# lucidrains/audiolm-pytorch

Measured on NVIDIA H100. Metric: CoarseTransformer tokens/sec fwd+bwd seq2048, higher is better.
Workload: dtype bf16

## Files before the change

audiolm_pytorch_b200/_lib.py:

```python
from __future__ import annotations

import ctypes as C
import os
from pathlib import Path

import torch

_PKG = Path(__file__).resolve().parent
LIB_PATH = _PKG / "libalm_b200.so"

P = C.c_void_p
I = C.c_int
L = C.c_int64
F = C.c_float
U32 = C.c_uint32
U64 = C.c_uint64
DROP = [F, U64, U32]

SIGNATURES: dict[str, list] = {
    "alm_gemm_bf16": [P, I, L, L, P, I, L, L, P, I, L, L, I, I, I, I, F, P, I, I, P],
    "alm_mqa_attn_fwd": [P, L, P, L, L, P, L, L, P, P, L, P, L, P, L, L, I, I, I, I, I, F, *DROP, P],
    "alm_mqa_attn_bwd": [P, L, P, L, L, P, L, L, P, L, P, P, P, I, P, L, P, P, L, P, L, P, P, L, L, I, I, I, I, I, F, *DROP,
                         P],
    "alm_pack_key_mask": [P, P, I, I, P],
# ... 36 lines not shown
    "alm_rvq_pack_codebooks": [P, P, P, L, I, P],
    "alm_rvq_prepare": [P, L, P, P, L, P, I, I, P],
    "alm_rvq_select": [P, L, P, P, P, P, L, P, P, L, I, I, I, I, P],
    "alm_rvq_decode": [P, L, P, P, L, I, I, I, I, P],
}


class AlmError(RuntimeError):
    pass


_lib = None


def load() -> C.CDLL:
    global _lib
    if _lib is not None:
        return _lib
    if not LIB_PATH.exists():
        raise AlmError(
            f"{LIB_PATH} not found. Build it with `python -m audiolm_pytorch_b200.build` "
            "(there is no CPU / PyTorch fallback for the hot path)."
        )
    lib = C.CDLL(str(LIB_PATH), mode=os.RTLD_LOCAL | os.RTLD_NOW)
    lib.alm_version.restype = I
    lib.alm_status_string.restype = C.c_char_p
    lib.alm_status_string.argtypes = [I]
    lib.alm_launch_count.restype = C.c_ulonglong
    lib.alm_reset_launch_count.restype = None
    lib.alm_decode_stack_scratch_bytes.restype = L
    lib.alm_decode_stack_scratch_bytes.argtypes = [I, I, I, I]
    lib.alm_gemm_head_ce_tiles.restype = I
    lib.alm_gemm_head_ce_tiles.argtypes = [I]
    lib.alm_decode_stack_grid.restype = I
    lib.alm_decode_stack_grid.argtypes = []
    lib.alm_decode_stack_plan.restype = I
    lib.alm_decode_stack_plan.argtypes = [I, I, I, I, I, P]
    lib.alm_decode_stack_trace_offset.restype = L
    lib.alm_decode_stack_trace_offset.argtypes = [I, I, I, I]
    for name, argtypes in SIGNATURES.items():
        fn = getattr(lib, name)
        fn.argtypes = argtypes
        fn.restype = I
    _lib = lib
    return lib


def ptr(t) -> int | None:
    if t is None:
        return None
    return t.data_ptr()


def stream_handle() -> int:
    return torch.cuda.current_stream().cuda_stream


def call(name: str, *args) -> None:
    lib = load()
    conv = []
    for a in args:
        if isinstance(a, torch.Tensor):
            if not a.is_cuda:
                raise AlmError(f"{name}: got a {a.device} tensor; the hot path has no CPU implementation")
            conv.append(a.data_ptr())
        else:
# ... 13 lines not shown
```

audiolm_pytorch_b200/csrc/gemm_wgmma.cu:

```cuda
#include "alm_common.cuh"
#include "ptx_sm90.cuh"

namespace alm {

struct GemmParams {
  void* C;
  const float* bias;
  long long ldc, strideC;
  int M, N, K, batch;
  int m_blocks, n_blocks, k_blocks, split_k;
  int c_fp32, acc_mode;
  int tma_store;
  float alpha;
  int ce_mode;
  const long long* ce_labels;
  long long ce_ignore;
  float* ce_part;
  float* ce_lab;
  const float* ce_lse;
  const float* ce_num;
  const float* ce_den;
};

constexpr int GEMM_BLOCK_M = 128;
constexpr int GEMM_BLOCK_K = 64;
constexpr int GEMM_THREADS = 384;

template <int BLOCK_N>
struct GemmCfg {
  static constexpr int STAGES = BLOCK_N == 256 ? 4 : (BLOCK_N == 128 ? 6 : 8);
  static constexpr int A_BYTES = GEMM_BLOCK_M * GEMM_BLOCK_K * 2;
  static constexpr int B_BYTES = BLOCK_N * GEMM_BLOCK_K * 2;
  static constexpr int C_SUB_BYTES = 64 * 64 * 2;
  static constexpr int C_STAGE_BYTES = 4 * C_SUB_BYTES;
  static constexpr int SMEM_BYTES =
      STAGES * (A_BYTES + B_BYTES) + C_STAGE_BYTES + 1024  + 256 ;
  static_assert(SMEM_BYTES <= 227 * 1024, "exceeds the sm_90 dynamic shared memory limit");
};

template <int BLOCK_N, bool A_MN, bool B_MN, bool CE = false>
__global__ void __launch_bounds__(GEMM_THREADS, 1)
gemm_bf16_wgmma_kernel(const __grid_constant__ CUtensorMap tmA, const __grid_constant__ CUtensorMap tmB,
                       const __grid_constant__ CUtensorMap tmC, const GemmParams p) {
  using Cfg = GemmCfg<BLOCK_N>;
  constexpr int STAGES = Cfg::STAGES;
  extern __shared__ uint8_t smem_raw[];
  uint8_t* smem = reinterpret_cast<uint8_t*>((reinterpret_cast<uintptr_t>(smem_raw) + 1023) & ~uintptr_t(1023));
  uint8_t* smem_a = smem;
  uint8_t* smem_b = smem + STAGES * Cfg::A_BYTES;
  uint8_t* stage_c = smem + STAGES * (Cfg::A_BYTES + Cfg::B_BYTES);
  uint64_t* bars = reinterpret_cast<uint64_t*>(stage_c + Cfg::C_STAGE_BYTES);
  uint64_t* full_bar = bars;
  uint64_t* empty_bar = bars + STAGES;

  const int warp = threadIdx.x >> 5;
  const int lane = threadIdx.x & 31;
  const int wg = warp >> 2;

  if (threadIdx.x == 0) {
    tma_prefetch_desc(&tmA);
    tma_prefetch_desc(&tmB);
    if (p.tma_store) tma_prefetch_desc(&tmC);
    for (int i = 0; i < STAGES; ++i) {
      mbar_init(&full_bar[i], 1);
      mbar_init(&empty_bar[i], 8);
    }
    fence_mbar_init();
  }
  __syncthreads();

  const int tiles_per_batch = p.m_blocks * p.n_blocks * p.split_k;
  const int total_tiles = tiles_per_batch * p.batch;
  const int kb_per_split = (p.k_blocks + p.split_k - 1) / p.split_k;

  auto decode = [&](int t, int& b, int& s, int& mb, int& nb) {
    b = t / tiles_per_batch;
    int r = t - b * tiles_per_batch;
    s = r / (p.m_blocks * p.n_blocks);
    r -= s * (p.m_blocks * p.n_blocks);
    mb = r / p.n_blocks;
    nb = r - mb * p.n_blocks;
  };
  auto k_range = [&](int s, int& kb0, int& kb1) {
    kb0 = s * kb_per_split;
    kb1 = min(p.k_blocks, kb0 + kb_per_split);
  };

  if (wg == 0) {
    setmaxnreg_dec<40>();
    if (warp == 0) {
      int stage = 0;
      uint32_t phase = 0;
      for (int t = blockIdx.x; t < total_tiles; t += gridDim.x) {
        int b, s, mb, nb, kb0, kb1;
        decode(t, b, s, mb, nb);
        k_range(s, kb0, kb1);
        const int m0 = mb * GEMM_BLOCK_M, n0 = nb * BLOCK_N;
        for (int kb = kb0; kb < kb1; ++kb) {
          mbar_wait(&empty_bar[stage], phase ^ 1u);
          uint8_t* sa = smem_a + stage * Cfg::A_BYTES;
          uint8_t* sb = smem_b + stage * Cfg::B_BYTES;
          const int k0 = kb * GEMM_BLOCK_K;
          if (elect_one_sync()) {
            mbar_arrive_expect_tx(&full_bar[stage], Cfg::A_BYTES + Cfg::B_BYTES);
            if constexpr (!A_MN) {
              tma_load_3d(sa, &tmA, &full_bar[stage], k0, m0, b);
            } else {
#pragma unroll
              for (int i = 0; i < GEMM_BLOCK_M / 64; ++i)
                tma_load_3d(sa + i * (GEMM_BLOCK_K * 128), &tmA, &full_bar[stage], m0 + i * 64, k0, b);
            }
            if constexpr (!B_MN) {
              tma_load_3d(sb, &tmB, &full_bar[stage], k0, n0, b);
            } else {
#pragma unroll
              for (int i = 0; i < BLOCK_N / 64; ++i)
                tma_load_3d(sb + i * (GEMM_BLOCK_K * 128), &tmB, &full_bar[stage], n0 + i * 64, k0, b);
            }
          }
          __syncwarp();
          if (++stage == STAGES) { stage = 0; phase ^= 1u; }
        }
      }
    }
    return;
  }

  setmaxnreg_inc<232>();
  const int cw = wg - 1;
  const int wq = warp & 3;
  const int r_base = cw * 64 + wq * 16 + (lane >> 2);
  const int c_lane = 2 * (lane & 3);
  int stage = 0;
  uint32_t phase = 0;
  float acc[BLOCK_N / 2];
  for (int t = blockIdx.x; t < total_tiles; t += gridDim.x) {
    int b, s, mb, nb, kb0, kb1;
    decode(t, b, s, mb, nb);
    k_range(s, kb0, kb1);
    int prev_stage = -1;
    for (int kb = kb0; kb < kb1; ++kb) {
      mbar_wait(&full_bar[stage], phase);
      const uint32_t a_addr = smem_u32(smem_a + stage * Cfg::A_BYTES) + cw * 8192;
      const uint32_t b_addr = smem_u32(smem_b + stage * Cfg::B_BYTES);
      wgmma_fence_acc(acc);
      wgmma_fence();
#pragma unroll
      for (int k = 0; k < GEMM_BLOCK_K / 16; ++k) {
        const uint64_t da = A_MN ? wgmma_desc_sw128(a_addr + k * 2048, 1024, GEMM_BLOCK_K * 128)
                                 : wgmma_desc_sw128(a_addr + k * 32, 1024, 16);
        const uint64_t db = B_MN ? wgmma_desc_sw128(b_addr + k * 2048, 1024, GEMM_BLOCK_K * 128)
                                 : wgmma_desc_sw128(b_addr + k * 32, 1024, 16);
        wgmma_ss<BLOCK_N, A_MN ? 1 : 0, B_MN ? 1 : 0>(acc, da, db, (kb > kb0 || k > 0) ? 1u : 0u);
      }
      wgmma_commit();
      wgmma_wait<1>();
      wgmma_fence_acc(acc);
      if (prev_stage >= 0 && lane == 0) mbar_arrive(&empty_bar[prev_stage]);
      prev_stage = stage;
      if (++stage == STAGES) { stage = 0; phase ^= 1u; }
    }
    wgmma_wait<0>();
    wgmma_fence_acc(acc);
    if (prev_stage >= 0 && lane == 0) mbar_arrive(&empty_bar[prev_stage]);

    const int n0 = nb * BLOCK_N;
    if constexpr (!CE) {
      if (p.tma_store) {
        constexpr int SUBS = BLOCK_N / 64, NBUF = SUBS % 2 == 0 ? 2 : 1;
        const uint32_t st_base =
            smem_u32(stage_c) + cw * 2 * Cfg::C_SUB_BYTES + (wq * 16 + (lane >> 2)) * 128 + (lane & 3) * 4;
#pragma unroll
        for (int sub = 0; sub < SUBS; ++sub) {
          uint8_t* buf = stage_c + (cw * 2 + sub % NBUF) * Cfg::C_SUB_BYTES;
          if ((threadIdx.x & 127) == 0) bulk_wait_group_read<NBUF - 1>();
          named_bar_sync(1 + cw, 128);
#pragma unroll
          for (int h = 0; h < 2; ++h)
#pragma unroll
            for (int jj = 0; jj < 8; ++jj) {
              const int j = sub * 8 + jj;
              const int col = n0 + 8 * j + c_lane;
              float v0 = acc[4 * j + 2 * h] * p.alpha, v1 = acc[4 * j + 2 * h + 1] * p.alpha;
              if (p.bias != nullptr) {
                if (col < p.N) v0 += __ldg(p.bias + col);
                if (col + 1 < p.N) v1 += __ldg(p.bias + col + 1);
              }
              st_shared_u32(st_base + (sub % NBUF) * Cfg::C_SUB_BYTES + h * 1024 + ((jj ^ (lane >> 2)) << 4),
                            pack_bf16x2(v0, v1));
            }
          fence_proxy_async_smem();
          named_bar_sync(1 + cw, 128);
          if ((threadIdx.x & 127) == 0) {
            tma_store_3d(&tmC, buf, n0 + sub * 64, mb * GEMM_BLOCK_M + cw * 64, b);
            bulk_commit_group();
          }
        }
        continue;
      }
    }

#pragma unroll
    for (int h = 0; h < 2; ++h) {
      const int gm = mb * GEMM_BLOCK_M + r_base + 8 * h;
      const bool row_ok = gm < p.M;
      const long long row_off = (long long)b * p.strideC + (long long)gm * p.ldc;
      [[maybe_unused]] float ce_lse2 = 0.f, ce_scale = 0.f;
      [[maybe_unused]] long long ce_label = -1;
      if constexpr (CE) {
        if (row_ok) {
          ce_label = p.ce_labels[gm];
          if (p.ce_mode == 2) {
            ce_lse2 = p.ce_lse[gm] * 1.4426950408889634f;
            ce_scale = ce_label == p.ce_ignore ? 0.f : __ldg(p.ce_num) / __ldg(p.ce_den);
          }
        }
        if (p.ce_mode == 1) {
          float cm = -INFINITY;
#pragma unroll
          for (int j = 0; j < BLOCK_N / 8; ++j)
#pragma unroll
            for (int c = 0; c < 2; ++c) {
              const int col = n0 + 8 * j + c_lane + c;
              float v = acc[4 * j + 2 * h + c] * p.alpha;
              if (p.bias != nullptr && col < p.N) v += __ldg(p.bias + col);
              if (row_ok && col == ce_label) p.ce_lab[gm] = v;
              v = col < p.N ? v * 1.4426950408889634f : -INFINITY;
              acc[4 * j + 2 * h + c] = v;
              cm = fmaxf(cm, v);
            }
          cm = fmaxf(cm, __shfl_xor_sync(0xffffffffu, cm, 1));
          cm = fmaxf(cm, __shfl_xor_sync(0xffffffffu, cm, 2));
          float cs = 0.f;
#pragma unroll
          for (int j = 0; j < BLOCK_N / 8; ++j)
#pragma unroll
            for (int c = 0; c < 2; ++c) cs += exp2f(acc[4 * j + 2 * h + c] - cm);
          cs += __shfl_xor_sync(0xffffffffu, cs, 1);
          cs += __shfl_xor_sync(0xffffffffu, cs, 2);
          if (row_ok && (lane & 3) == 0) {
            float* pp = p.ce_part + ((size_t)gm * p.n_blocks + nb) * 2;
            pp[0] = cm;
            pp[1] = cs;
          }
          continue;
        }
      }
      if (!row_ok) continue;
#pragma unroll
      for (int j = 0; j < BLOCK_N / 8; ++j) {
        const int col = n0 + 8 * j + c_lane;
        if (col >= p.N) break;
        float v0 = acc[4 * j + 2 * h] * p.alpha, v1 = acc[4 * j + 2 * h + 1] * p.alpha;
        const bool pair = col + 1 < p.N;
        if (p.bias != nullptr) {
          v0 += __ldg(p.bias + col);
          if (pair) v1 += __ldg(p.bias + col + 1);
        }
        if constexpr (CE) {
          v0 = (exp2f(v0 * 1.4426950408889634f - ce_lse2) - (col == ce_label ? 1.f : 0.f)) * ce_scale;
          v1 = (exp2f(v1 * 1.4426950408889634f - ce_lse2) - (col + 1 == ce_label ? 1.f : 0.f)) * ce_scale;
        }
        if (p.c_fp32) {
          float* dst = reinterpret_cast<float*>(p.C) + row_off + col;
          const bool vec = pair && ((reinterpret_cast<uintptr_t>(dst) & 7u) == 0);
          if (p.acc_mode == 2) {
            if (vec) {
              asm volatile("red.global.add.v2.f32 [%0], {%1, %2};" ::"l"(dst), "f"(v0), "f"(v1) : "memory");
            } else {
              atomicAdd(dst, v0);
              if (pair) atomicAdd(dst + 1, v1);
            }
          } else if (vec) {
            float2 o = make_float2(v0, v1);
            if (p.acc_mode == 1) {
              const float2 old = *reinterpret_cast<float2*>(dst);
              o.x += old.x; o.y += old.y;
            }
            *reinterpret_cast<float2*>(dst) = o;
          } else {
            dst[0] = (p.acc_mode == 1 ? dst[0] : 0.f) + v0;
            if (pair) dst[1] = (p.acc_mode == 1 ? dst[1] : 0.f) + v1;
          }
        } else {
          __nv_bfloat16* dst = reinterpret_cast<__nv_bfloat16*>(p.C) + row_off + col;
          if (p.acc_mode != 0) {
            v0 += __bfloat162float(dst[0]);
            if (pair) v1 += __bfloat162float(dst[1]);
          }
          if (pair && ((reinterpret_cast<uintptr_t>(dst) & 3u) == 0)) {
            *reinterpret_cast<uint32_t*>(dst) = pack_bf16x2(v0, v1);
          } else {
            dst[0] = __float2bfloat16_rn(v0);
            if (pair) dst[1] = __float2bfloat16_rn(v1);
          }
        }
      }
    }
  }
  if ((threadIdx.x & 127) == 0) bulk_wait_group<0>();
}

template <int BLOCK_N, bool A_MN, bool B_MN, bool CE = false>
static int launch_gemm(const CUtensorMap& tmA, const CUtensorMap& tmB, const CUtensorMap& tmC, const GemmParams& p,
                       cudaStream_t stream) {
  using Cfg = GemmCfg<BLOCK_N>;
  auto kfn = gemm_bf16_wgmma_kernel<BLOCK_N, A_MN, B_MN, CE>;
  static bool attr_set = false;
  if (!attr_set) {
    ALM_CUDA_OK(cudaFuncSetAttribute(kfn, cudaFuncAttributeMaxDynamicSharedMemorySize, Cfg::SMEM_BYTES));
    attr_set = true;
  }
  const int total = p.m_blocks * p.n_blocks * p.split_k * p.batch;
  const int grid = total < num_sms() ? total : num_sms();
  kfn<<<grid, GEMM_THREADS, Cfg::SMEM_BYTES, stream>>>(tmA, tmB, tmC, p);
  ALM_CHECK_LAUNCH();
  ALM_LAUNCHED(1);
  return ALM_OK;
}

static int pick_block_n(int N) {
  if (N <= 64) return 64;
  if (N <= 128) return 128;
  const int pad256 = ceil_div(N, 256) * 256, pad128 = ceil_div(N, 128) * 128;
  return (pad128 * 10 < pad256 * 9) ? 128 : 256;
}

}

namespace alm {
struct CeEpilogue {
  int mode;
  const long long* labels;
  long long ignore;
  float* part;
  float* lab;
  const float* lse;
  const float* num;
  const float* den;
};
}

static int gemm_common(const void* A, int a_mn, int64_t lda, int64_t strideA, const void* B, int b_mn, int64_t ldb,
                       int64_t strideB, void* C, int c_fp32, int64_t ldc, int64_t strideC, int M, int N, int K, int batch,
                       float alpha, const float* bias, int acc_mode, int split_k, cudaStream_t stream,
                       const alm::CeEpilogue* ce) {
  using namespace alm;
  ALM_REQUIRE(A && B && (C || (ce && ce->mode == 1)), ALM_ERR_ARG);
  ALM_REQUIRE(M > 0 && N > 0 && K > 0 && batch > 0, ALM_ERR_ARG);
  ALM_REQUIRE(acc_mode >= 0 && acc_mode <= 2 && split_k >= 1, ALM_ERR_ARG);
  ALM_REQUIRE(split_k == 1 || (acc_mode == 2 && c_fp32), ALM_ERR_ARG);
  ALM_REQUIRE(!(a_mn && !b_mn), ALM_ERR_UNSUPPORTED);
  ALM_REQUIRE(lda % 8 == 0 && ldb % 8 == 0 && strideA % 8 == 0 && strideB % 8 == 0, ALM_ERR_ALIGN);

  const int BN = pick_block_n(N);
  GemmParams p;
  p.C = C;
  p.bias = bias;
  p.ldc = ldc;
  p.strideC = strideC;
  p.M = M; p.N = N; p.K = K; p.batch = batch;
  p.m_blocks = ceil_div(M, GEMM_BLOCK_M);
  p.n_blocks = ceil_div(N, BN);
  p.k_blocks = ceil_div(K, GEMM_BLOCK_K);
  if (split_k > p.k_blocks) split_k = p.k_blocks;
  while (split_k > 1 && (split_k - 1) * ceil_div(p.k_blocks, split_k) >= p.k_blocks) --split_k;
  p.split_k = split_k;
  p.c_fp32 = c_fp32;
  p.acc_mode = acc_mode;
  p.alpha = alpha;
  p.ce_mode = 0;
  if (ce != nullptr) {
    p.ce_mode = ce->mode;
    p.ce_labels = ce->labels;
    p.ce_ignore = ce->ignore;
    p.ce_part = ce->part;
    p.ce_lab = ce->lab;
    p.ce_lse = ce->lse;
    p.ce_num = ce->num;
    p.ce_den = ce->den;
  }

  CUtensorMap tmA, tmB;
  {
    uint64_t dims[3], strides[3];
    uint32_t box[3];
    if (!a_mn) {
      dims[0] = (uint64_t)K; dims[1] = (uint64_t)M;
      box[0] = GEMM_BLOCK_K; box[1] = GEMM_BLOCK_M;
    } else {
      dims[0] = (uint64_t)M; dims[1] = (uint64_t)K;
      box[0] = 64; box[1] = GEMM_BLOCK_K;
    }
    dims[2] = (uint64_t)batch; box[2] = 1;
    strides[0] = 2; strides[1] = (uint64_t)lda * 2;
    strides[2] = batch > 1 ? (uint64_t)strideA * 2 : dims[1] * strides[1];
    int rc = make_tensor_map(&tmA, A, 2, 3, dims, strides, box, true);
    if (rc != ALM_OK) return rc;
  }
  {
    uint64_t dims[3], strides[3];
    uint32_t box[3];
    if (!b_mn) {
      dims[0] = (uint64_t)K; dims[1] = (uint64_t)N;
      box[0] = GEMM_BLOCK_K; box[1] = (uint32_t)BN;
    } else {
      dims[0] = (uint64_t)N; dims[1] = (uint64_t)K;
      box[0] = 64; box[1] = GEMM_BLOCK_K;
    }
    dims[2] = (uint64_t)batch; box[2] = 1;
    strides[0] = 2; strides[1] = (uint64_t)ldb * 2;
    strides[2] = batch > 1 ? (uint64_t)strideB * 2 : dims[1] * strides[1];
    int rc = make_tensor_map(&tmB, B, 2, 3, dims, strides, box, true);
    if (rc != ALM_OK) return rc;
  }

  CUtensorMap tmC = {};
  p.tma_store = ce == nullptr && !c_fp32 && acc_mode == 0 && (reinterpret_cast<uintptr_t>(C) & 15u) == 0 &&
                (ldc * 2) % 16 == 0 && (batch == 1 || (strideC * 2) % 16 == 0);
  if (p.tma_store) {
    const uint64_t dims[3] = {(uint64_t)N, (uint64_t)M, (uint64_t)batch};
    const uint64_t strides[3] = {2, (uint64_t)ldc * 2, batch > 1 ? (uint64_t)strideC * 2 : (uint64_t)M * ldc * 2};
    const uint32_t box[3] = {64, 64, 1};
    int rc = make_tensor_map(&tmC, C, 2, 3, dims, strides, box, true);
    if (rc != ALM_OK) return rc;
  }

  if (ce != nullptr) {
    if (BN == 256) return launch_gemm<256, false, false, true>(tmA, tmB, tmC, p, stream);
    if (BN == 128) return launch_gemm<128, false, false, true>(tmA, tmB, tmC, p, stream);
    return launch_gemm<64, false, false, true>(tmA, tmB, tmC, p, stream);
  }
#define ALM_GEMM_DISPATCH(BN_)                                                             \
  if (!a_mn && !b_mn) return launch_gemm<BN_, false, false>(tmA, tmB, tmC, p, stream);     \
  if (!a_mn && b_mn) return launch_gemm<BN_, false, true>(tmA, tmB, tmC, p, stream);       \
  return launch_gemm<BN_, true, true>(tmA, tmB, tmC, p, stream);
  if (BN == 256) { ALM_GEMM_DISPATCH(256) }
  if (BN == 128) { ALM_GEMM_DISPATCH(128) }
  { ALM_GEMM_DISPATCH(64) }
#undef ALM_GEMM_DISPATCH
}

extern "C" int alm_gemm_bf16(const void* A, int a_mn, int64_t lda, int64_t strideA, const void* B, int b_mn,
                             int64_t ldb, int64_t strideB, void* C, int c_fp32, int64_t ldc, int64_t strideC, int M,
                             int N, int K, int batch, float alpha, const float* bias, int acc_mode, int split_k,
                             alm_stream_t stream_) {
  return gemm_common(A, a_mn, lda, strideA, B, b_mn, ldb, strideB, C, c_fp32, ldc, strideC, M, N, K, batch, alpha, bias,
                     acc_mode, split_k, reinterpret_cast<cudaStream_t>(stream_), nullptr);
}

extern "C" int alm_gemm_head_ce_tiles(int V) { return alm::ceil_div(V, alm::pick_block_n(V)); }

extern "C" int alm_gemm_head_ce(const void* X, int64_t ldx, const void* W, int64_t ldw, const float* bias,
                                const int64_t* labels, int64_t ignore_index, int mode, float* part, float* lab_logit,
                                const float* lse, const float* scale_num, const float* scale_den, void* dlogits,
                                int64_t ldd, int M, int V, int K, alm_stream_t stream_) {
  ALM_REQUIRE(mode == 1 || mode == 2, ALM_ERR_ARG);
  ALM_REQUIRE(labels != nullptr, ALM_ERR_ARG);
  if (mode == 1) ALM_REQUIRE(part && lab_logit, ALM_ERR_ARG);
  else ALM_REQUIRE(lse && scale_num && scale_den && dlogits && ldd >= V, ALM_ERR_ARG);
  alm::CeEpilogue ce{mode, reinterpret_cast<const long long*>(labels), (long long)ignore_index, part, lab_logit, lse,
                     scale_num, scale_den};
  return gemm_common(X, 0, ldx, 0, W, 0, ldw, 0, dlogits, 0, ldd, 0, M, V, K, 1, 1.f, bias, 0, 1,
                     reinterpret_cast<cudaStream_t>(stream_), &ce);
}
```

audiolm_pytorch_b200/csrc/ptx_sm90.cuh:

```cuda
#pragma once
#include <cuda.h>
#include <cuda_runtime.h>
#include <cuda_bf16.h>
#include <stdint.h>
#include <stdio.h>

namespace alm {

__device__ __forceinline__ uint32_t smem_u32(const void* p) {
  return static_cast<uint32_t>(__cvta_generic_to_shared(p));
}
__device__ __forceinline__ uint32_t lane_id() { return threadIdx.x & 31u; }

__device__ __forceinline__ uint64_t global_timer_ns() {
  uint64_t t;
  asm volatile("mov.u64 %0, %%globaltimer;" : "=l"(t));
  return t;
}

__device__ __forceinline__ void mbar_init(uint64_t* bar, uint32_t arrive_count) {
  asm volatile("mbarrier.init.shared::cta.b64 [%0], %1;" ::"r"(smem_u32(bar)), "r"(arrive_count) : "memory");
}
__device__ __forceinline__ void fence_mbar_init() {
  asm volatile("fence.mbarrier_init.release.cluster;" ::: "memory");
// ... 55 lines not shown
      ::"r"(smem_u32(smem_dst)), "l"(reinterpret_cast<uint64_t>(m)), "r"(smem_u32(bar)), "r"(c0), "r"(c1), "r"(c2)
      : "memory");
}
__device__ __forceinline__ void tma_store_3d(const CUtensorMap* m, const void* smem_src, int32_t c0, int32_t c1,
                                             int32_t c2) {
  asm volatile("cp.async.bulk.tensor.3d.global.shared::cta.bulk_group [%0, {%2, %3, %4}], [%1];"
               ::"l"(reinterpret_cast<uint64_t>(m)), "r"(smem_u32(smem_src)), "r"(c0), "r"(c1), "r"(c2)
               : "memory");
}
__device__ __forceinline__ void tma_reduce_add_3d(const CUtensorMap* m, uint32_t smem_src, int32_t c0, int32_t c1,
                                                  int32_t c2) {
  asm volatile("cp.reduce.async.bulk.tensor.3d.global.shared::cta.add.bulk_group [%0, {%2, %3, %4}], [%1];"
               ::"l"(reinterpret_cast<uint64_t>(m)), "r"(smem_src), "r"(c0), "r"(c1), "r"(c2)
               : "memory");
}
__device__ __forceinline__ void bulk_commit_group() { asm volatile("cp.async.bulk.commit_group;" ::: "memory"); }
template <int N>
__device__ __forceinline__ void bulk_wait_group_read() {
  asm volatile("cp.async.bulk.wait_group.read %0;" ::"n"(N) : "memory");
}
template <int N>
__device__ __forceinline__ void bulk_wait_group() {
  asm volatile("cp.async.bulk.wait_group %0;" ::"n"(N) : "memory");
}
__device__ __forceinline__ void st_shared_u32(uint32_t smem_addr, uint32_t v) {
  asm volatile("st.shared.u32 [%0], %1;" ::"r"(smem_addr), "r"(v) : "memory");
}
__device__ __forceinline__ void st_shared_f32x2(uint32_t smem_addr, float a, float b) {
  asm volatile("st.shared.v2.f32 [%0], {%1, %2};" ::"r"(smem_addr), "f"(a), "f"(b) : "memory");
}
__device__ __forceinline__ void named_bar_sync(uint32_t id, uint32_t nthreads) {
  asm volatile("bar.sync %0, %1;" ::"r"(id), "r"(nthreads) : "memory");
}
__device__ __forceinline__ uint64_t wgmma_desc_sw128(uint32_t smem_addr, uint32_t sbo_bytes, uint32_t lbo_bytes) {
  uint32_t lo = ((smem_addr >> 4) & 0x3FFFu) | (((lbo_bytes >> 4) & 0x3FFFu) << 16);
  uint32_t hi = ((sbo_bytes >> 4) & 0x3FFFu) | (1u << 30);
  return (static_cast<uint64_t>(hi) << 32) | lo;
}
__device__ __forceinline__ uint64_t wgmma_desc_nosw(uint32_t smem_addr, uint32_t sbo_bytes, uint32_t lbo_bytes) {
  uint32_t lo = ((smem_addr >> 4) & 0x3FFFu) | (((lbo_bytes >> 4) & 0x3FFFu) << 16);
  uint32_t hi = ((sbo_bytes >> 4) & 0x3FFFu);
  return (static_cast<uint64_t>(hi) << 32) | lo;
}
__device__ __forceinline__ void wgmma_fence() { asm volatile("wgmma.fence.sync.aligned;" ::: "memory"); }
__device__ __forceinline__ void wgmma_commit() { asm volatile("wgmma.commit_group.sync.aligned;" ::: "memory"); }
template <int N>
__device__ __forceinline__ void wgmma_wait() {
  asm volatile("wgmma.wait_group.sync.aligned %0;" ::"n"(N) : "memory");
}
template <int R>
__device__ __forceinline__ void wgmma_fence_acc(float (&d)[R]) {
#pragma unroll
  for (int i = 0; i < R; ++i) asm volatile("" : "+f"(d[i])::"memory");
}
template <int N>
__device__ __forceinline__ void setmaxnreg_inc() {
  asm volatile("setmaxnreg.inc.sync.aligned.u32 %0;" ::"n"(N));
}
template <int N>
__device__ __forceinline__ void setmaxnreg_dec() {
  asm volatile("setmaxnreg.dec.sync.aligned.u32 %0;" ::"n"(N));
}

template <int TA, int TB>
__device__ __forceinline__ void wgmma_ss_n32(float (&d)[16], uint64_t da, uint64_t db, uint32_t accumulate) {
  asm volatile(
// ... 103 lines not shown
```

audiolm_pytorch_b200/ops.py:

```python
from __future__ import annotations

import ctypes
import functools

import torch

from . import _lib

_SMS: dict[int, int] = {}


def num_sms(device=None) -> int:
    idx = None if device is None else torch.device(device).index
    if idx is None:
        idx = torch.cuda.current_device()
    if idx not in _SMS:
        _SMS[idx] = torch.cuda.get_device_properties(idx).multi_processor_count
    return _SMS[idx]


bf16 = torch.bfloat16
f32 = torch.float32


# ... 57 lines not shown
    assert a3.stride(-1) == 1 and b3.stride(-1) == 1
    nb = a3.shape[0]
    assert b3.shape[0] == nb
    if a_mn:
        K, M = a3.shape[1], a3.shape[2]
    else:
        M, K = a3.shape[1], a3.shape[2]
    if b_mn:
        Kb, N = b3.shape[1], b3.shape[2]
    else:
        N, Kb = b3.shape[1], b3.shape[2]
    assert K == Kb, f"K mismatch {K} vs {Kb}"
    if out is None:
        out = torch.empty((nb, M, N) if batched else (M, N), device=a.device, dtype=out_dtype)
        assert acc_mode == 0
    o3 = out.unsqueeze(0) if out.dim() == 2 else out
    assert o3.shape == (nb, M, N) and o3.stride(-1) == 1
    assert o3.dtype in (bf16, f32)
    if bias is not None:
        assert bias.dtype == f32 and bias.numel() == N and bias.is_contiguous()
    if _PROFILE is not None and PROFILE_SHAPES:
        cls += f" M{M} N{N} K{K} b{nb} {'mn' if a_mn else 'k'}{'mn' if b_mn else 'k'} s{split_k}"
    with _timed(cls, 2.0 * M * N * K * nb):
        _lib.call(
            "alm_gemm_bf16",
            a3, int(a_mn), a3.stride(1), a3.stride(0) if nb > 1 else 0,
            b3, int(b_mn), b3.stride(1), b3.stride(0) if nb > 1 else 0,
            o3, int(o3.dtype == f32), o3.stride(1), o3.stride(0) if nb > 1 else 0,
            M, N, K, nb, float(alpha), bias, int(acc_mode), int(split_k),
        )
    return out


def _check_bias(bias, heads, n_q, n_k):
    assert bias.dtype == f32 and bias.dim() == 3 and bias.shape[0] == heads and bias.shape[1] == n_q
    assert bias.shape[2] >= n_k and bias.stride(2) == 1 and bias.stride(1) % 4 == 0 and bias.stride(0) % 4 == 0
    return bias.stride(0), bias.stride(1)


def _ptr_array(tensors):
    import ctypes
    arr = (ctypes.c_void_p * len(tensors))(*[t.data_ptr() for t in tensors])
    return arr


def embed_gather(src, tables, d):
    _check_cuda(src, *tables)
    assert src.dtype == torch.int32 and src.is_contiguous() and src.shape[1] == 2
    assert all(t.dtype == f32 and t.is_contiguous() and t.shape[-1] == d for t in tables)
    M = src.shape[0]
    out = torch.empty(M, d, device=src.device, dtype=f32)
    import ctypes
    _lib.call("alm_embed_gather", ctypes.cast(_ptr_array(tables), ctypes.c_void_p), len(tables), src, out, M, d)
    return out


def embed_scatter(src, grad_tables, dout):
    _check_cuda(src, dout, *grad_tables)
    M, d = dout.shape
    assert dout.dtype == f32 and dout.is_contiguous()
    import ctypes
    _lib.call("alm_embed_scatter", ctypes.cast(_ptr_array(grad_tables), ctypes.c_void_p), len(grad_tables), src, dout,
              M, d)


class PackedKeyMask:
# ... 654 lines not shown
```

audiolm_pytorch_b200/transformer.py:

```python
from __future__ import annotations

import torch
from torch import nn

from . import ops

bf16 = torch.bfloat16
f32 = torch.float32


def exists(v):
    return v is not None


def default(v, d):
    return v if exists(v) else d


def _pad8(n: int) -> int:
    return (n + 7) // 8 * 8


def _check_dropout(p, name="dropout"):
    if not 0.0 <= float(p) < 1.0:
# ... 113 lines not shown
        self._cache = {}
        self.generation = 0

    def clear(self):
        self._cache.clear()
        self.generation += 1

    def get(self, key, params, build):
        ver = tuple((p.data_ptr(), p._version) for p in params)
        hit = self._cache.get(key)
        if hit is not None and hit[0] == ver:
            return hit[1]
        with torch.inference_mode(False), torch.no_grad():
            val = build()
        self._cache[key] = (ver, val)
        return val


def pack_plain(w):
    return ops.cast_pad(w.detach(), _pad8(w.shape[1]))


def pack_w1(w, inner):
    ip = _pad8(inner)
    out = torch.zeros(2 * ip, w.shape[1], device=w.device, dtype=bf16)
    ops.cast_pad(w.detach()[:inner], out=out[:inner])
    ops.cast_pad(w.detach()[inner:], out=out[ip:ip + inner])
    return out


def best_split_k(M, N, K, n_sm=None):
    if n_sm is None:
        n_sm = ops.num_sms() if torch.cuda.is_available() else 132
    bn = 64 if N <= 64 else (128 if N <= 128 or (-(-N // 128) * 128) * 10 < (-(-N // 256) * 256) * 9 else 256)
    tiles = -(-M // 128) * -(-N // bn)
    kb = -(-K // 64)
    best, best_t = 1, None
    for s in range(1, min(64, kb) + 1):
        t = -(-tiles * s // n_sm) * (-(-kb // s) + 6)
        if best_t is None or t < best_t:
            best, best_t = s, t
    return best


def wgrad(dy, x, out):
    Mtok = dy.shape[0]
    s = best_split_k(dy.shape[1], x.shape[1], Mtok)
    ops.gemm(dy, x, a_mn=True, b_mn=True, out=out, acc_mode=2 if s > 1 else 1, split_k=s)


class _StackFn(torch.autograd.Function):

    @staticmethod
    def forward(ctx, tr, x, mask, bias, drop, want_kv, *params):
        out, kv, saved = tr._walk_forward(x, mask, bias, drop, save=any(ctx.needs_input_grad), want_kv=want_kv)
        ctx.tr = tr
        ctx.saved = saved
        ctx.bias_grad = bias is not None and ctx.needs_input_grad[3]
        ctx.mark_non_differentiable(kv)
        return out, kv

    @staticmethod
    def backward(ctx, dout, _dkv):
        tr = ctx.tr
        S = ctx.saved
        S["dbias"] = torch.zeros_like(S["bias"]) if ctx.bias_grad else None
        dx, grads = tr._walk_backward(S, dout)
        dbias = S["dbias"]
        ctx.saved = None
        return (None, dx, None, dbias, None, None, *grads)


# ... 387 lines not shown
```

include/alm_b200.h:

```cpp
#ifndef ALM_B200_H_
#define ALM_B200_H_

#include <stddef.h>
#include <stdint.h>

#ifdef __cplusplus
extern "C" {
#endif

typedef struct CUstream_st* alm_stream_t;

typedef enum alm_status {
  ALM_OK = 0,
  ALM_ERR_ARG = -1,
  ALM_ERR_ALIGN = -2,
  ALM_ERR_CUDA = -3,
  ALM_ERR_UNSUPPORTED = -4
} alm_status;

int alm_version(void);
const char* alm_status_string(int code);
unsigned long long alm_launch_count(void);
void alm_reset_launch_count(void);

int alm_gemm_bf16(const void* A, int a_mn, int64_t lda, int64_t strideA, const void* B, int b_mn, int64_t ldb,
                  int64_t strideB, void* C, int c_fp32, int64_t ldc, int64_t strideC, int M, int N, int K, int batch,
                  float alpha, const float* bias, int acc_mode, int split_k, alm_stream_t stream);

int alm_embed_gather(const float* const* tables, int n_tables, const int32_t* src, float* out, int M, int d,
                     alm_stream_t stream);
int alm_embed_scatter(float* const* grad_tables, int n_tables, const int32_t* src, const float* dout, int M, int d,
                      alm_stream_t stream);
int alm_pack_key_mask(const void* key_mask, void* bits, int b, int n_k, alm_stream_t stream);
int alm_mqa_attn_fwd(const void* q, int64_t ldq, const void* k, int64_t ldk, int64_t k_bstride, const void* v,
                     int64_t ldv, int64_t v_bstride, const void* key_mask, void* o, int64_t ldo, float* lse,
                     int64_t lse_stride, const float* bias, int64_t bias_hstride, int64_t bias_rstride, int b, int h,
                     int n_q, int n_k, int causal, float scale, float dropout_p, uint64_t seed, uint32_t site,
                     alm_stream_t stream);

int alm_mqa_attn_bwd(const void* q, int64_t ldq, const void* k, int64_t ldk, int64_t k_bstride, const void* v,
                     int64_t ldv, int64_t v_bstride, const void* d_o, int64_t lddo, const void* key_mask,
                     const float* lse, const float* delta, int n_q_pad, void* dq, int64_t lddq, float* dq_acc,
                     void* dk, int64_t lddk, void* dv, int64_t lddv, const float* bias, float* dbias,
                     int64_t bias_hstride, int64_t bias_rstride, int b, int h, int n_q, int n_k, int causal,
                     float scale, float dropout_p, uint64_t seed, uint32_t site, alm_stream_t stream);
int alm_attn_delta(const void* o, int64_t ldo, const void* d_o, int64_t lddo, float* delta ,
                   int64_t delta_stride, float* dq_acc, int b, int h, int n, alm_stream_t stream);

int alm_bias_gather_fwd(const float* table, const int32_t* idx, const float* override_h, float* out, int heads,
                        int n_q, int n_k, int64_t ld, alm_stream_t stream);
int alm_bias_gather_bwd(const float* dbias, const int32_t* idx, float* dtable, float* doverride, int heads, int n_q,
                        int n_k, int64_t ld, alm_stream_t stream);

int alm_gemv_bf16(const void* x, int64_t ldx, const void* W, int64_t ldw, void* out, int c_fp32, int64_t ldo,
                  const float* bias, int rows, int N, int K, alm_stream_t stream);
int alm_kv_append(const void* kv_new, int64_t ld, void* k_cache, void* v_cache, int64_t cache_bstride,
                  const int32_t* len, int max_len, int b, alm_stream_t stream);
int alm_mqa_attn_decode(const void* q, int64_t ldq, const void* k_cache, const void* v_cache, int64_t cache_bstride,
                        const int32_t* len, int max_len, const void* key_mask, int64_t mask_bstride, const float* bias,
                        int64_t bias_ld, void* o, int64_t ldo,
// ... 105 lines not shown
```

Before: 752,800.

## Add ping-pong warpgroup GEMM variant for short-K bf16 TMA-store GEMMs

```diff
diff --git a/audiolm_pytorch_b200/_lib.py b/audiolm_pytorch_b200/_lib.py
--- a/audiolm_pytorch_b200/_lib.py
+++ b/audiolm_pytorch_b200/_lib.py
@@ -92,6 +92,10 @@
     lib.alm_decode_stack_scratch_bytes.argtypes = [I, I, I, I]
     lib.alm_gemm_head_ce_tiles.restype = I
     lib.alm_gemm_head_ce_tiles.argtypes = [I]
+    lib.alm_gemm_plan.restype = I
+    lib.alm_gemm_plan.argtypes = [I, I, I, I, I, P, P, P]
+    lib.alm_gemm_select_kernel.restype = I
+    lib.alm_gemm_select_kernel.argtypes = [I]
     lib.alm_decode_stack_grid.restype = I
     lib.alm_decode_stack_grid.argtypes = []
     lib.alm_decode_stack_plan.restype = I
diff --git a/audiolm_pytorch_b200/csrc/gemm_wgmma.cu b/audiolm_pytorch_b200/csrc/gemm_wgmma.cu
--- a/audiolm_pytorch_b200/csrc/gemm_wgmma.cu
+++ b/audiolm_pytorch_b200/csrc/gemm_wgmma.cu
@@ -38,10 +38,11 @@
   static_assert(SMEM_BYTES <= 227 * 1024, "exceeds the sm_90 dynamic shared memory limit");
 };
 
-template <int BLOCK_N, bool A_MN, bool B_MN, bool CE = false>
+template <int BLOCK_N, bool A_MN, bool B_MN, bool CE = false, bool PP = false>
 __global__ void __launch_bounds__(GEMM_THREADS, 1)
 gemm_bf16_wgmma_kernel(const __grid_constant__ CUtensorMap tmA, const __grid_constant__ CUtensorMap tmB,
                        const __grid_constant__ CUtensorMap tmC, const GemmParams p) {
+  static_assert(!PP || (BLOCK_N == 128 && !CE), "the ping-pong kernel has 128 x 128 tiles and no CE epilogue");
   using Cfg = GemmCfg<BLOCK_N>;
   constexpr int STAGES = Cfg::STAGES;
   extern __shared__ uint8_t smem_raw[];
@@ -63,7 +64,7 @@
     if (p.tma_store) tma_prefetch_desc(&tmC);
     for (int i = 0; i < STAGES; ++i) {
       mbar_init(&full_bar[i], 1);
-      mbar_init(&empty_bar[i], 8);
+      mbar_init(&empty_bar[i], PP ? 4 : 8);
     }
     fence_mbar_init();
   }
@@ -127,82 +128,110 @@
   }
 
   setmaxnreg_inc<232>();
+  constexpr int MH = PP ? 2 : 1;
   const int cw = wg - 1;
   const int wq = warp & 3;
-  const int r_base = cw * 64 + wq * 16 + (lane >> 2);
+  const int row0 = PP ? 0 : cw * 64;
+  const int r_base = row0 + wq * 16 + (lane >> 2);
   const int c_lane = 2 * (lane & 3);
   int stage = 0;
   uint32_t phase = 0;
-  float acc[BLOCK_N / 2];
-  for (int t = blockIdx.x; t < total_tiles; t += gridDim.x) {
+  float acc[MH][BLOCK_N / 2];
+  int i = 0;
+  for (int t = blockIdx.x; t < total_tiles; t += gridDim.x, ++i) {
     int b, s, mb, nb, kb0, kb1;
     decode(t, b, s, mb, nb);
     k_range(s, kb0, kb1);
+    if constexpr (PP) {
+      if ((i & 1) != cw) {
+        const int adv = stage + (kb1 - kb0);
+        phase ^= (uint32_t)(adv / STAGES) & 1u;
+        stage = adv % STAGES;
+        continue;
+      }
+      if (i > 0) named_bar_sync(3 + cw, 256);
+    }
     int prev_stage = -1;
     for (int kb = kb0; kb < kb1; ++kb) {
       mbar_wait(&full_bar[stage], phase);
-      const uint32_t a_addr = smem_u32(smem_a + stage * Cfg::A_BYTES) + cw * 8192;
+      const uint32_t a_addr = smem_u32(smem_a + stage * Cfg::A_BYTES) + row0 * 128;
       const uint32_t b_addr = smem_u32(smem_b + stage * Cfg::B_BYTES);
-      wgmma_fence_acc(acc);
+#pragma unroll
+      for (int mh = 0; mh < MH; ++mh) wgmma_fence_acc(acc[mh]);
       wgmma_fence();
 #pragma unroll
       for (int k = 0; k < GEMM_BLOCK_K / 16; ++k) {
-        const uint64_t da = A_MN ? wgmma_desc_sw128(a_addr + k * 2048, 1024, GEMM_BLOCK_K * 128)
-                                 : wgmma_desc_sw128(a_addr + k * 32, 1024, 16);
         const uint64_t db = B_MN ? wgmma_desc_sw128(b_addr + k * 2048, 1024, GEMM_BLOCK_K * 128)
                                  : wgmma_desc_sw128(b_addr + k * 32, 1024, 16);
-        wgmma_ss<BLOCK_N, A_MN ? 1 : 0, B_MN ? 1 : 0>(acc, da, db, (kb > kb0 || k > 0) ? 1u : 0u);
+#pragma unroll
+        for (int mh = 0; mh < MH; ++mh) {
+          const uint32_t am = a_addr + mh * 8192;
+          const uint64_t da = A_MN ? wgmma_desc_sw128(am + k * 2048, 1024, GEMM_BLOCK_K * 128)
+                                   : wgmma_desc_sw128(am + k * 32, 1024, 16);
+          wgmma_ss<BLOCK_N, A_MN ? 1 : 0, B_MN ? 1 : 0>(acc[mh], da, db, (kb > kb0 || k > 0) ? 1u : 0u);
+        }
       }
       wgmma_commit();
       wgmma_wait<1>();
-      wgmma_fence_acc(acc);
+#pragma unroll
+      for (int mh = 0; mh < MH; ++mh) wgmma_fence_acc(acc[mh]);
       if (prev_stage >= 0 && lane == 0) mbar_arrive(&empty_bar[prev_stage]);
       prev_stage = stage;
       if (++stage == STAGES) { stage = 0; phase ^= 1u; }
     }
+    if constexpr (PP) {
+      if (t + gridDim.x < total_tiles) named_bar_arrive(3 + (cw ^ 1), 256);
+    }
     wgmma_wait<0>();
-    wgmma_fence_acc(acc);
+#pragma unroll
+    for (int mh = 0; mh < MH; ++mh) wgmma_fence_acc(acc[mh]);
     if (prev_stage >= 0 && lane == 0) mbar_arrive(&empty_bar[prev_stage]);
 
     const int n0 = nb * BLOCK_N;
     if constexpr (!CE) {
       if (p.tma_store) {
-        constexpr int SUBS = BLOCK_N / 64, NBUF = SUBS % 2 == 0 ? 2 : 1;
+        constexpr int SUBS = BLOCK_N / 64, NBUF = (MH * SUBS) % 2 == 0 ? 2 : 1;
         const uint32_t st_base =
             smem_u32(stage_c) + cw * 2 * Cfg::C_SUB_BYTES + (wq * 16 + (lane >> 2)) * 128 + (lane & 3) * 4;
 #pragma unroll
-        for (int sub = 0; sub < SUBS; ++sub) {
-          uint8_t* buf = stage_c + (cw * 2 + sub % NBUF) * Cfg::C_SUB_BYTES;
-          if ((threadIdx.x & 127) == 0) bulk_wait_group_read<NBUF - 1>();
-          named_bar_sync(1 + cw, 128);
-#pragma unroll
-          for (int h = 0; h < 2; ++h)
-#pragma unroll
-            for (int jj = 0; jj < 8; ++jj) {
-              const int j = sub * 8 + jj;
-              const int col = n0 + 8 * j + c_lane;
-              float v0 = acc[4 * j + 2 * h] * p.alpha, v1 = acc[4 * j + 2 * h + 1] * p.alpha;
-              if (p.bias != nullptr) {
-                if (col < p.N) v0 += __ldg(p.bias + col);
-                if (col + 1 < p.N) v1 += __ldg(p.bias + col + 1);
+        for (int mh = 0; mh < MH; ++mh)
+#pragma unroll
+          for (int sub = 0; sub < SUBS; ++sub) {
+            const int box = mh * SUBS + sub;
+            uint8_t* buf = stage_c + (cw * 2 + box % NBUF) * Cfg::C_SUB_BYTES;
+            if ((threadIdx.x & 127) == 0) bulk_wait_group_read<NBUF - 1>();
+            named_bar_sync(1 + cw, 128);
+#pragma unroll
+            for (int h = 0; h < 2; ++h)
+#pragma unroll
+              for (int jj = 0; jj < 8; ++jj) {
+                const int j = sub * 8 + jj;
+                const int col = n0 + 8 * j + c_lane;
+                float v0 = acc[mh][4 * j + 2 * h] * p.alpha, v1 = acc[mh][4 * j + 2 * h + 1] * p.alpha;
+                if (p.bias != nullptr) {
+                  if (col < p.N) v0 += __ldg(p.bias + col);
+                  if (col + 1 < p.N) v1 += __ldg(p.bias + col + 1);
+                }
+                st_shared_u32(st_base + (box % NBUF) * Cfg::C_SUB_BYTES + h * 1024 + ((jj ^ (lane >> 2)) << 4),
+                              pack_bf16x2(v0, v1));
               }
-              st_shared_u32(st_base + (sub % NBUF) * Cfg::C_SUB_BYTES + h * 1024 + ((jj ^ (lane >> 2)) << 4),
-                            pack_bf16x2(v0, v1));
+            fence_proxy_async_smem();
+            named_bar_sync(1 + cw, 128);
+            if ((threadIdx.x & 127) == 0) {
+              tma_store_3d(&tmC, buf, n0 + sub * 64, mb * GEMM_BLOCK_M + row0 + mh * 64, b);
+              bulk_commit_group();
             }
-          fence_proxy_async_smem();
-          named_bar_sync(1 + cw, 128);
-          if ((threadIdx.x & 127) == 0) {
-            tma_store_3d(&tmC, buf, n0 + sub * 64, mb * GEMM_BLOCK_M + cw * 64, b);
-            bulk_commit_group();
-          }
-        }
+          }
         continue;
       }
     }
 
 #pragma unroll
+    for (int mh = 0; mh < MH; ++mh)
+#pragma unroll
     for (int h = 0; h < 2; ++h) {
-      const int gm = mb * GEMM_BLOCK_M + r_base + 8 * h;
+      float (&a)[BLOCK_N / 2] = acc[mh];
+      const int gm = mb * GEMM_BLOCK_M + r_base + 64 * mh + 8 * h;
       const bool row_ok = gm < p.M;
       const long long row_off = (long long)b * p.strideC + (long long)gm * p.ldc;
       [[maybe_unused]] float ce_lse2 = 0.f, ce_scale = 0.f;
@@ -222,11 +251,11 @@
 #pragma unroll
             for (int c = 0; c < 2; ++c) {
               const int col = n0 + 8 * j + c_lane + c;
-              float v = acc[4 * j + 2 * h + c] * p.alpha;
+              float v = a[4 * j + 2 * h + c] * p.alpha;
               if (p.bias != nullptr && col < p.N) v += __ldg(p.bias + col);
               if (row_ok && col == ce_label) p.ce_lab[gm] = v;
               v = col < p.N ? v * 1.4426950408889634f : -INFINITY;
-              acc[4 * j + 2 * h + c] = v;
+              a[4 * j + 2 * h + c] = v;
               cm = fmaxf(cm, v);
             }
           cm = fmaxf(cm, __shfl_xor_sync(0xffffffffu, cm, 1));
@@ -235,7 +264,7 @@
 #pragma unroll
           for (int j = 0; j < BLOCK_N / 8; ++j)
 #pragma unroll
-            for (int c = 0; c < 2; ++c) cs += exp2f(acc[4 * j + 2 * h + c] - cm);
+            for (int c = 0; c < 2; ++c) cs += exp2f(a[4 * j + 2 * h + c] - cm);
           cs += __shfl_xor_sync(0xffffffffu, cs, 1);
           cs += __shfl_xor_sync(0xffffffffu, cs, 2);
           if (row_ok && (lane & 3) == 0) {
@@ -251,7 +280,7 @@
       for (int j = 0; j < BLOCK_N / 8; ++j) {
         const int col = n0 + 8 * j + c_lane;
         if (col >= p.N) break;
-        float v0 = acc[4 * j + 2 * h] * p.alpha, v1 = acc[4 * j + 2 * h + 1] * p.alpha;
+        float v0 = a[4 * j + 2 * h] * p.alpha, v1 = a[4 * j + 2 * h + 1] * p.alpha;
         const bool pair = col + 1 < p.N;
         if (p.bias != nullptr) {
           v0 += __ldg(p.bias + col);
@@ -301,11 +330,11 @@
   if ((threadIdx.x & 127) == 0) bulk_wait_group<0>();
 }
 
-template <int BLOCK_N, bool A_MN, bool B_MN, bool CE = false>
+template <int BLOCK_N, bool A_MN, bool B_MN, bool CE = false, bool PP = false>
 static int launch_gemm(const CUtensorMap& tmA, const CUtensorMap& tmB, const CUtensorMap& tmC, const GemmParams& p,
                        cudaStream_t stream) {
   using Cfg = GemmCfg<BLOCK_N>;
-  auto kfn = gemm_bf16_wgmma_kernel<BLOCK_N, A_MN, B_MN, CE>;
+  auto kfn = gemm_bf16_wgmma_kernel<BLOCK_N, A_MN, B_MN, CE, PP>;
   static bool attr_set = false;
   if (!attr_set) {
     ALM_CUDA_OK(cudaFuncSetAttribute(kfn, cudaFuncAttributeMaxDynamicSharedMemorySize, Cfg::SMEM_BYTES));
@@ -324,6 +353,27 @@
   if (N <= 128) return 128;
   const int pad256 = ceil_div(N, 256) * 256, pad128 = ceil_div(N, 128) * 128;
   return (pad128 * 10 < pad256 * 9) ? 128 : 256;
+}
+
+enum { GEMM_OUT_TMA = 0, GEMM_OUT_REG = 1, GEMM_OUT_CE = 2 };
+struct GemmPlan {
+  bool pingpong;
+  int block_n;
+};
+static int g_gemm_kernel = 0;
+
+static GemmPlan plan_gemm(int M, int N, int K, int split_k, int out_kind) {
+  (void)M;
+  if (out_kind == GEMM_OUT_CE || g_gemm_kernel == 1) return {false, pick_block_n(N)};
+  if (g_gemm_kernel == 2) return {true, 128};
+  const bool pingpong = out_kind == GEMM_OUT_TMA && split_k == 1 && K <= 1024 && N > 128 && N <= 1024;
+  return pingpong ? GemmPlan{true, 128} : GemmPlan{false, pick_block_n(N)};
+}
+
+static int clamp_split_k(int k_blocks, int split_k) {
+  if (split_k > k_blocks) split_k = k_blocks;
+  while (split_k > 1 && (split_k - 1) * ceil_div(k_blocks, split_k) >= k_blocks) --split_k;
+  return split_k;
 }
 
 }
@@ -353,7 +403,11 @@
   ALM_REQUIRE(!(a_mn && !b_mn), ALM_ERR_UNSUPPORTED);
   ALM_REQUIRE(lda % 8 == 0 && ldb % 8 == 0 && strideA % 8 == 0 && strideB % 8 == 0, ALM_ERR_ALIGN);
 
-  const int BN = pick_block_n(N);
+  const bool tma_store = ce == nullptr && !c_fp32 && acc_mode == 0 && (reinterpret_cast<uintptr_t>(C) & 15u) == 0 &&
+                         (ldc * 2) % 16 == 0 && (batch == 1 || (strideC * 2) % 16 == 0);
+  const GemmPlan plan =
+      plan_gemm(M, N, K, split_k, ce != nullptr ? GEMM_OUT_CE : (tma_store ? GEMM_OUT_TMA : GEMM_OUT_REG));
+  const int BN = plan.block_n;
   GemmParams p;
   p.C = C;
   p.bias = bias;
@@ -363,9 +417,7 @@
   p.m_blocks = ceil_div(M, GEMM_BLOCK_M);
   p.n_blocks = ceil_div(N, BN);
   p.k_blocks = ceil_div(K, GEMM_BLOCK_K);
-  if (split_k > p.k_blocks) split_k = p.k_blocks;
-  while (split_k > 1 && (split_k - 1) * ceil_div(p.k_blocks, split_k) >= p.k_blocks) --split_k;
-  p.split_k = split_k;
+  p.split_k = clamp_split_k(p.k_blocks, split_k);
   p.c_fp32 = c_fp32;
   p.acc_mode = acc_mode;
   p.alpha = alpha;
@@ -416,8 +468,7 @@
   }
 
   CUtensorMap tmC = {};
-  p.tma_store = ce == nullptr && !c_fp32 && acc_mode == 0 && (reinterpret_cast<uintptr_t>(C) & 15u) == 0 &&
-                (ldc * 2) % 16 == 0 && (batch == 1 || (strideC * 2) % 16 == 0);
+  p.tma_store = tma_store;
   if (p.tma_store) {
     const uint64_t dims[3] = {(uint64_t)N, (uint64_t)M, (uint64_t)batch};
     const uint64_t strides[3] = {2, (uint64_t)ldc * 2, batch > 1 ? (uint64_t)strideC * 2 : (uint64_t)M * ldc * 2};
@@ -431,14 +482,35 @@
     if (BN == 128) return launch_gemm<128, false, false, true>(tmA, tmB, tmC, p, stream);
     return launch_gemm<64, false, false, true>(tmA, tmB, tmC, p, stream);
   }
-#define ALM_GEMM_DISPATCH(BN_)                                                             \
-  if (!a_mn && !b_mn) return launch_gemm<BN_, false, false>(tmA, tmB, tmC, p, stream);     \
-  if (!a_mn && b_mn) return launch_gemm<BN_, false, true>(tmA, tmB, tmC, p, stream);       \
-  return launch_gemm<BN_, true, true>(tmA, tmB, tmC, p, stream);
-  if (BN == 256) { ALM_GEMM_DISPATCH(256) }
-  if (BN == 128) { ALM_GEMM_DISPATCH(128) }
-  { ALM_GEMM_DISPATCH(64) }
+#define ALM_GEMM_DISPATCH(BN_, PP_)                                                                    \
+  if (!a_mn && !b_mn) return launch_gemm<BN_, false, false, false, PP_>(tmA, tmB, tmC, p, stream);     \
+  if (!a_mn && b_mn) return launch_gemm<BN_, false, true, false, PP_>(tmA, tmB, tmC, p, stream);       \
+  return launch_gemm<BN_, true, true, false, PP_>(tmA, tmB, tmC, p, stream);
+  if (plan.pingpong) { ALM_GEMM_DISPATCH(128, true) }
+  if (BN == 256) { ALM_GEMM_DISPATCH(256, false) }
+  if (BN == 128) { ALM_GEMM_DISPATCH(128, false) }
+  { ALM_GEMM_DISPATCH(64, false) }
 #undef ALM_GEMM_DISPATCH
+}
+
+extern "C" int alm_gemm_plan(int M, int N, int K, int split_k, int out_kind, int* pingpong, int* block_n,
+                             int* tiles) {
+  using namespace alm;
+  ALM_REQUIRE(M > 0 && N > 0 && K > 0 && split_k >= 1 && out_kind >= 0 && out_kind <= 2, ALM_ERR_ARG);
+  ALM_REQUIRE(pingpong && block_n && tiles, ALM_ERR_ARG);
+  const GemmPlan plan = plan_gemm(M, N, K, split_k, out_kind);
+  *pingpong = plan.pingpong ? 1 : 0;
+  *block_n = plan.block_n;
+  *tiles = ceil_div(M, GEMM_BLOCK_M) * ceil_div(N, plan.block_n) *
+           clamp_split_k(ceil_div(K, GEMM_BLOCK_K), split_k);
+  return ALM_OK;
+}
+
+extern "C" int alm_gemm_select_kernel(int which) {
+  if (which < 0 || which > 2) return -1;
+  const int prev = alm::g_gemm_kernel;
+  alm::g_gemm_kernel = which;
+  return prev;
 }
 
 extern "C" int alm_gemm_bf16(const void* A, int a_mn, int64_t lda, int64_t strideA, const void* B, int b_mn,
@@ -449,7 +521,9 @@
                      acc_mode, split_k, reinterpret_cast<cudaStream_t>(stream_), nullptr);
 }
 
-extern "C" int alm_gemm_head_ce_tiles(int V) { return alm::ceil_div(V, alm::pick_block_n(V)); }
+extern "C" int alm_gemm_head_ce_tiles(int V) {
+  return alm::ceil_div(V, alm::plan_gemm(1, V, 1, 1, alm::GEMM_OUT_CE).block_n);
+}
 
 extern "C" int alm_gemm_head_ce(const void* X, int64_t ldx, const void* W, int64_t ldw, const float* bias,
                                 const int64_t* labels, int64_t ignore_index, int mode, float* part, float* lab_logit,
diff --git a/audiolm_pytorch_b200/csrc/ptx_sm90.cuh b/audiolm_pytorch_b200/csrc/ptx_sm90.cuh
--- a/audiolm_pytorch_b200/csrc/ptx_sm90.cuh
+++ b/audiolm_pytorch_b200/csrc/ptx_sm90.cuh
@@ -111,6 +111,9 @@
 __device__ __forceinline__ void named_bar_sync(uint32_t id, uint32_t nthreads) {
   asm volatile("bar.sync %0, %1;" ::"r"(id), "r"(nthreads) : "memory");
 }
+__device__ __forceinline__ void named_bar_arrive(uint32_t id, uint32_t nthreads) {
+  asm volatile("bar.arrive %0, %1;" ::"r"(id), "r"(nthreads) : "memory");
+}
 __device__ __forceinline__ uint64_t wgmma_desc_sw128(uint32_t smem_addr, uint32_t sbo_bytes, uint32_t lbo_bytes) {
   uint32_t lo = ((smem_addr >> 4) & 0x3FFFu) | (((lbo_bytes >> 4) & 0x3FFFu) << 16);
   uint32_t hi = ((sbo_bytes >> 4) & 0x3FFFu) | (1u << 30);
diff --git a/audiolm_pytorch_b200/ops.py b/audiolm_pytorch_b200/ops.py
--- a/audiolm_pytorch_b200/ops.py
+++ b/audiolm_pytorch_b200/ops.py
@@ -113,6 +113,24 @@
     return out
 
 
+GEMM_OUT_TMA, GEMM_OUT_REG, GEMM_OUT_CE = 0, 1, 2
+_GEMM_KERNELS = {"auto": 0, "cooperative": 1, "pingpong": 2}
+
+
+def gemm_plan(M, N, K, split_k=1, out_kind=GEMM_OUT_TMA):
+    pp, bn, tiles = ctypes.c_int(), ctypes.c_int(), ctypes.c_int()
+    rc = _lib.load().alm_gemm_plan(int(M), int(N), int(K), int(split_k), int(out_kind), ctypes.byref(pp),
+                                   ctypes.byref(bn), ctypes.byref(tiles))
+    if rc != 0:
+        raise _lib.AlmError(f"alm_gemm_plan({M}, {N}, {K}, {split_k}, {out_kind}) failed ({rc})")
+    return bool(pp.value), bn.value, tiles.value
+
+
+def gemm_select_kernel(which="auto"):
+    prev = _lib.load().alm_gemm_select_kernel(_GEMM_KERNELS[which])
+    return {v: k for k, v in _GEMM_KERNELS.items()}[prev]
+
+
 def _check_bias(bias, heads, n_q, n_k):
     assert bias.dtype == f32 and bias.dim() == 3 and bias.shape[0] == heads and bias.shape[1] == n_q
     assert bias.shape[2] >= n_k and bias.stride(2) == 1 and bias.stride(1) % 4 == 0 and bias.stride(0) % 4 == 0
diff --git a/audiolm_pytorch_b200/transformer.py b/audiolm_pytorch_b200/transformer.py
--- a/audiolm_pytorch_b200/transformer.py
+++ b/audiolm_pytorch_b200/transformer.py
@@ -169,12 +169,16 @@
 def best_split_k(M, N, K, n_sm=None):
     if n_sm is None:
         n_sm = ops.num_sms() if torch.cuda.is_available() else 132
-    bn = 64 if N <= 64 else (128 if N <= 128 or (-(-N // 128) * 128) * 10 < (-(-N // 256) * 256) * 9 else 256)
+    pingpong, bn, _ = ops.gemm_plan(M, N, K, 1, ops.GEMM_OUT_REG)
     tiles = -(-M // 128) * -(-N // bn)
     kb = -(-K // 64)
     best, best_t = 1, None
     for s in range(1, min(64, kb) + 1):
-        t = -(-tiles * s // n_sm) * (-(-kb // s) + 6)
+        rounds = -(-tiles * s // n_sm)
+        if pingpong:
+            t = rounds * (-(-kb // s) + 1) + 6
+        else:
+            t = rounds * (-(-kb // s) + 6)
         if best_t is None or t < best_t:
             best, best_t = s, t
     return best
diff --git a/include/alm_b200.h b/include/alm_b200.h
--- a/include/alm_b200.h
+++ b/include/alm_b200.h
@@ -26,6 +26,8 @@
 int alm_gemm_bf16(const void* A, int a_mn, int64_t lda, int64_t strideA, const void* B, int b_mn, int64_t ldb,
                   int64_t strideB, void* C, int c_fp32, int64_t ldc, int64_t strideC, int M, int N, int K, int batch,
                   float alpha, const float* bias, int acc_mode, int split_k, alm_stream_t stream);
+int alm_gemm_plan(int M, int N, int K, int split_k, int out_kind, int* pingpong, int* block_n, int* tiles);
+int alm_gemm_select_kernel(int which);
 
 int alm_embed_gather(const float* const* tables, int n_tables, const int32_t* src, float* out, int M, int d,
                      alm_stream_t stream);
```

Measured after the change: 761,100, median of 6. No clear change (+1.1%).
